# choderalab/openmmtools

Hardware: NVIDIA B200
Metric: replica-exchange iterations/sec, 256-replica alchemical LJ fluid (higher is better)
Workload: dtype f32 dynamics, f64 energies and mixing

## Files before the change

openmmtools_b200/csrc/rx_walk2.cuh:

```cuda
#pragma once

struct SlotRec2 {
    uint32_t ij;
    uint32_t backmask;
    uint32_t lu_next;
    uint32_t alts;
};

#define W2_LOOKBACK 48

__device__ __forceinline__ double slot_logU(const uint32_t *__restrict__ words, unsigned s) {
    const double U = mt_double(words[2 * (size_t)s], words[2 * (size_t)s + 1]);
    return (U == 0.0) ? LOGU_ZERO : log(U);
}

__global__ void __launch_bounds__(256) k_slots_build2(const uint32_t *__restrict__ words, long long nslots, uint32_t mask,
                                                      SlotRec2 *__restrict__ rec) {
    __shared__ uint32_t s_ij[256 + W2_LOOKBACK];
    const long long s0 = (long long)blockIdx.x * 256;
    const int t = threadIdx.x;
    for (int q = t; q < 256 + W2_LOOKBACK; q += 256) {
        const long long s = s0 - W2_LOOKBACK + q;
        uint32_t ij = 0xffffffffu;
        if (s >= 0 && s < nslots) ij = (words[2 * s] & mask) | ((words[2 * s + 1] & mask) << 16);
        s_ij[q] = ij;
    }
    __syncthreads();
    const long long s = s0 + t;
    if (s >= nslots) return;
    const uint32_t ij = s_ij[t + W2_LOOKBACK];
    const uint32_t i = ij & 0xffffu, j = ij >> 16;
    uint32_t bm = 0, a1i = i, a1j = j;
    bool fi = false, fj = false;
#pragma unroll 4
    for (int b = 0; b < W2_LOOKBACK - 1; b++) {
        const uint32_t o = s_ij[t + W2_LOOKBACK - 1 - b];
        const uint32_t oi = o & 0xffffu, oj = o >> 16;
        const bool valid = (o != 0xffffffffu);
        if (b < 31) {
            const bool hit = valid && (oi == i || oi == j || oj == i || oj == j);
            bm |= (hit ? 1u : 0u) << (31 - b);
        }
        if (valid && oi != oj) {
            if (!fi && (oi == i || oj == i)) { a1i = (oi == i) ? oj : oi; fi = true; }
            if (!fj && (oi == j || oj == j)) { a1j = (oi == j) ? oj : oi; fj = true; }
        }
    }
    SlotRec2 r;
    r.ij = ij;
    r.backmask = bm;
    float lu = 0.f;
    if (s + 1 < nslots) lu = (float)slot_logU(words, (unsigned)(s + 1));
    r.lu_next = __float_as_uint(lu);
    r.alts = (a1i & 0xffu) | ((a1j & 0xffu) << 8);
    rec[s] = r;
}

__device__ __forceinline__ void w2_filter(float d_i, float f_ij, float d_j, float f_ji, float e0, float lu,
                                          bool &ge0, bool &acc, bool &undecided) {
    const float lp = (d_i - f_ij) + (d_j - f_ji);
    const float eps = fmaf(fabsf(f_ij) + fabsf(f_ji), 3.2e-5f, e0);
    ge0 = lp > eps;
    const float d = lp - lu;
    const float mar = fmaf(fabsf(lp) + fabsf(lu), 1.3e-7f, eps);
    const bool dec_lp = fabsf(lp) > eps;
    acc = ge0 || (dec_lp && d > mar);
    undecided = !(ge0 || (dec_lp && fabsf(d) > mar));
}

struct __align__(8) W2Replica {
    int state;
    float diag;
};

__device__ __forceinline__ float w2_image(const unsigned short *__restrict__ s_qhi, const unsigned char *__restrict__ s_qlo, unsigned a) {
    return __uint_as_float(__byte_perm((unsigned)s_qhi[a], (unsigned)s_qlo[a], 0x1045));
}

__device__ __forceinline__ uint2 w2_lds64(unsigned a) {
    uint2 v;
    asm volatile("ld.shared.v2.u32 {%0, %1}, [%2];" : "=r"(v.x), "=r"(v.y) : "r"(a) : "memory");
    return v;
}
__device__ __forceinline__ float w2_lds_f32(unsigned a) {
    float v;
    asm("ld.shared.f32 %0, [%1];" : "=f"(v) : "r"(a));
    return v;
}
__device__ __forceinline__ uint4 w2_lds128(unsigned a) {
    uint4 v;
    asm volatile("ld.shared.v4.u32 {%0, %1, %2, %3}, [%4];" : "=r"(v.x), "=r"(v.y), "=r"(v.z), "=r"(v.w) : "r"(a) : "memory");
    return v;
}
__device__ __forceinline__ uint4 w2_lds128_ctx(unsigned a) {
    uint4 v;
    asm("ld.shared.v4.u32 {%0, %1, %2, %3}, [%4];" : "=r"(v.x), "=r"(v.y), "=r"(v.z), "=r"(v.w) : "r"(a));
    return v;
}
__device__ __forceinline__ void w2_sts64(unsigned a, unsigned x, unsigned y) {
    asm volatile("st.shared.v2.u32 [%0], {%1, %2};" ::"r"(a), "r"(x), "r"(y) : "memory");
}
__device__ __forceinline__ unsigned w2_lds32(unsigned a) {
    unsigned v;
    asm volatile("ld.shared.u32 %0, [%1];" : "=r"(v) : "r"(a) : "memory");
    return v;
}
__device__ __forceinline__ float w2_image_at(unsigned a_hi, unsigned a_lo) {
    unsigned hi, lo;
    asm("ld.shared.u16 %0, [%1];" : "=r"(hi) : "r"(a_hi));
    asm("ld.shared.u8 %0, [%1];" : "=r"(lo) : "r"(a_lo));
    return __uint_as_float(__byte_perm(hi, lo, 0x1045));
}

#define W2_RING 512
__device__ __forceinline__ void w2_cp_async16(unsigned dst, const void *src) {
    asm volatile("cp.async.cg.shared.global [%0], [%1], 16;" ::"r"(dst), "l"(src) : "memory");
}
__device__ __forceinline__ void w2_cp_async_commit() { asm volatile("cp.async.commit_group;" ::: "memory"); }
template <int N>
__device__ __forceinline__ void w2_cp_async_wait() { asm volatile("cp.async.wait_group %0;" ::"n"(N) : "memory"); }

__device__ __noinline__ unsigned w2_exact_decision(const SlotRec2 *__restrict__ rec, const uint32_t *__restrict__ words,
                                                   const double *__restrict__ u, unsigned s, unsigned si, unsigned sj, int logK) {
    const unsigned ij = rec[s].ij;
    const unsigned rowi = (ij & 0xffffu) << logK, rowj = (ij >> 16) << logK;
    const double logp = swap_logp(u[rowi | sj], u[rowj | si], u[rowi | si], u[rowj | sj]);
    if (logp >= 0.0) return 3u;
    const unsigned s1 = s + 1;
    const double dd = logp - slot_logU(words, s1);
    bool acc;
    if (dd > 1e-9) acc = true;
    else if (dd < -1e-9) acc = false;
    else acc = mt_double(words[2 * (size_t)s1], words[2 * (size_t)s1 + 1]) < rx_exp_cr(logp);
    return acc ? 2u : 0u;
}

#define W2_THREADS 128
__global__ void __launch_bounds__(W2_THREADS) k_mix_walk2(const SlotRec2 *__restrict__ rec, const uint32_t *__restrict__ words,
                                                  unsigned nslots, const double *__restrict__ u, int K, int logK,
                                                  int *__restrict__ perm_g, uint32_t *__restrict__ slot_log,
                                                  const unsigned char *__restrict__ filt,
                                                  const double *__restrict__ filt_rowabs, MixCtl *ctl) {
    extern __shared__ uint4 s_w2[];
    __shared__ unsigned long long s_ptrs[2];
    uint4 *s_ring = s_w2;
    W2Replica *s_rep = (W2Replica *)(s_ring + W2_RING);
    unsigned char *s_q = (unsigned char *)(s_rep + K);
    const int tid = threadIdx.x, lane = tid & 31, warp = __shfl_sync(0xffffffffu, tid >> 5, 0);
    {
        const unsigned short *ghi = (const unsigned short *)filt;
        const unsigned char *glo = filt + 2 * (size_t)K * K;
        if (K >= 16) {
            const uint4 *ghi4 = (const uint4 *)ghi, *glo4 = (const uint4 *)glo;
            for (int q = tid; q < (K * K) / 8; q += W2_THREADS) {
                const int e = q * 8, row = e >> logK, col = e & (K - 1);
                *(uint4 *)(s_q + (size_t)3 * K * row + 2 * col) = ghi4[q];
            }
            for (int q = tid; q < (K * K) / 16; q += W2_THREADS) {
                const int e = q * 16, row = e >> logK, col = e & (K - 1);
                *(uint4 *)(s_q + (size_t)3 * K * row + 2 * K + col) = glo4[q];
            }
        } else {
            for (int q = tid; q < K * K; q += W2_THREADS) {
                const int row = q >> logK, col = q & (K - 1);
                unsigned char *rowp = s_q + (size_t)3 * K * row;
                ((unsigned short *)rowp)[col] = ghi[q];
                rowp[2 * K + col] = glo[q];
            }
        }
    }
    if (tid == 0) { s_ptrs[0] = (unsigned long long)__cvta_generic_to_global(slot_log); s_ptrs[1] = (unsigned long long)rec; }
    __syncthreads();
    float rowabs_max = 0.f;
    for (int q = tid; q < K; q += W2_THREADS) {
        W2Replica e;
        e.state = perm_g[q];
        const unsigned char *rowp = s_q + (size_t)3 * K * q;
        e.diag = __uint_as_float(__byte_perm((unsigned)((const unsigned short *)rowp)[e.state], (unsigned)rowp[2 * K + e.state], 0x1045));
        s_rep[q] = e;
    }
    for (int q = lane; q < K; q += 32)
        rowabs_max = fmaxf(rowabs_max, __fmul_ru(1.6e-14f, __fadd_ru(__double2float_ru(fabs(filt_rowabs[q])), 0.5f)));
    for (int o = 16; o; o >>= 1) rowabs_max = fmaxf(rowabs_max, __shfl_xor_sync(0xffffffffu, rowabs_max, o));
    const float eps_rows = __fadd_ru(__fadd_ru(rowabs_max, rowabs_max), 1e-9f);
    __syncthreads();
    if (warp != 0) return;
    const uint4 *__restrict__ recs = (const uint4 *)rec;

    const unsigned head0 = (unsigned)ctl->head;
    unsigned h = head0;
    const long long remaining0 = ctl->remaining;
    unsigned rem = remaining0 > 0x7fffffffLL ? 0x7fffffffu : (unsigned)remaining0;
    const unsigned rem0 = rem;
    unsigned rounds = 0, slow = 0;
    const unsigned h_end = nslots >= 1200u ? nslots - 560u : 0u;
    if (rem >= 130 && nslots >= 1200u && h + 99u <= h_end) {
        const unsigned ring_base = __shfl_sync(0xffffffffu, (unsigned)__cvta_generic_to_shared((const void *)s_ring), 0);
        const unsigned rep_base = __shfl_sync(0xffffffffu, (unsigned)__cvta_generic_to_shared((const void *)s_rep), 0);
        const unsigned img_base = __shfl_sync(0xffffffffu, (unsigned)__cvta_generic_to_shared((const void *)s_q), 0);
        const unsigned row_bytes = 3u * (unsigned)K, lo_off = 2u * (unsigned)K;
        unsigned r = h & 31u;
        unsigned w = ((unsigned)lane - h) & 31u;
        unsigned sA = h + w;
        const uint2 pl = w2_lds64((unsigned)__cvta_generic_to_shared((const void *)&s_ptrs[0]));
        const uint2 pr = w2_lds64((unsigned)__cvta_generic_to_shared((const void *)&s_ptrs[1]));
        const unsigned long long slot_log_r = ((unsigned long long)pl.y << 32) | pl.x;
        const uint4 *recs_r = (const uint4 *)(((unsigned long long)pr.y << 32) | pr.x);
        unsigned bmA, neqA, rowiA, rowjA, repiA, repjA;
        float luA, epsA;
        unsigned iB, jB, repiB, repjB;
        auto ahead = [&](const uint4 q) {
            iB = q.x & 0xffffu; jB = q.x >> 16;
            repiB = rep_base + (iB << 3); repjB = rep_base + (jB << 3);
        };
        auto derive = [&](const uint4 q, unsigned &bm, float &lu, float &eps, unsigned &neq, unsigned &rowi, unsigned &rowj,
                          unsigned &repi, unsigned &repj) {
            const unsigned i = q.x & 0xffffu, j = q.x >> 16;
            bm = q.y; lu = __uint_as_float(q.z);
            neq = i != j ? 0xffffffffu : 0u;
            eps = i != j ? eps_rows : -1e30f;
            rowi = img_base + i * row_bytes; rowj = img_base + j * row_bytes;
            repi = rep_base + (i << 3); repj = rep_base + (j << 3);
        };
        for (unsigned k = 0; k < 16u; k++) w2_cp_async16(ring_base + (((sA + 32u * k) & (W2_RING - 1)) << 4), recs + (sA + 32u * k));
        w2_cp_async_commit();
        w2_cp_async_wait<0>();
        __syncwarp();
        derive(w2_lds128(ring_base + ((sA & (W2_RING - 1)) << 4)), bmA, luA, epsA, neqA, rowiA, rowjA, repiA, repjA);
        unsigned ridxB = (sA + 32u) & (W2_RING - 1);
        uint4 qB = w2_lds128(ring_base + (ridxB << 4));
        ahead(qB);
        uint2 ei = w2_lds64(repiA), ej = w2_lds64(repjA);
        unsigned p_cm = 0, p_below = 0, p_chg = 0, p_entry = 0;
        float f_ij = 0.f, f_ji = 0.f;
        auto commit = [&]() {
            const unsigned p_advance = (unsigned)__popc(p_below);
            const unsigned bit = 1u << w;
            const bool p_mine = (p_cm & bit) != 0u;
            const bool p_swaps = (p_cm & bit & p_chg) != 0u;
            const bool p_promoted = (p_below & bit) != 0u;
            if (p_swaps) {
                w2_sts64(repiA, ej.x, __float_as_uint(f_ij));
                w2_sts64(repjA, ei.x, __float_as_uint(f_ji));
            }
            __syncwarp();
            const uint2 ein = w2_lds64(p_promoted ? repiB : repiA), ejn = w2_lds64(p_promoted ? repjB : repjA);
            if (p_mine)
                asm volatile("st.global.u32 [%0], %1;" ::"l"(slot_log_r + 4ull * sA), "r"(p_entry) : "memory");
            if (p_promoted) {
                bmA = qB.y; luA = __uint_as_float(qB.z);
                neqA = iB != jB ? 0xffffffffu : 0u;
                epsA = iB != jB ? eps_rows : -1e30f;
                rowiA = img_base + iB * row_bytes; rowjA = img_base + jB * row_bytes;
                repiA = repiB; repjA = repjB;
                sA += 32u;
                w2_cp_async16(ring_base + (((ridxB - 32u) & (W2_RING - 1)) << 4), recs_r + (sA + 480u));
                ridxB = (ridxB + 32u) & (W2_RING - 1);
            }
            w2_cp_async_commit();
            qB = w2_lds128(ring_base + (ridxB << 4));
            h += p_advance;
            r = (r + p_advance) & 31u;
            rem -= __popc(p_cm);
            ei = ein;
            ej = ejn;
            w = (w - p_advance) & 31u;
        };
        unsigned Cw = 0;
        float bias = 0.f, lu_saved = 0.f;
        bool injected = false;
        for (;;) {
            if (rem < 130u || h + 99u > h_end) break;
            unsigned quota = min(min((rem - 97u) >> 5, (h_end - h - 66u) >> 5), injected ? 1u : 64u);
            do {
                commit();
                rounds++;
                const unsigned si = ei.x, sj = ej.x;
                f_ij = w2_image_at(rowiA + 2u * sj, rowiA + lo_off + sj);
                f_ji = w2_image_at(rowjA + 2u * si, rowjA + lo_off + si);
                const float e0 = fmaf(fabsf(__uint_as_float(ei.y)) + fabsf(__uint_as_float(ej.y)), 3.2e-5f, epsA);
                w2_cp_async_wait<8>();
                ahead(qB);
                bool ge0, acc, undecided;
                w2_filter(__uint_as_float(ei.y), f_ij, __uint_as_float(ej.y) + bias, f_ji, e0, luA, ge0, acc, undecided);
                const unsigned und = undecided ? 1u : 0u;
                const bool changes = acc && neqA != 0u;
                const unsigned G = __ballot_sync(0xffffffffu, ge0);
                const unsigned A = __ballot_sync(0xffffffffu, changes);
                const unsigned Gw = __funnelshift_r(G, G, r), Aw = __funnelshift_r(A, A, r);
                const unsigned X = ~Gw;
                const unsigned starts = X & ~(X << 1);
                const unsigned SE = starts & 0x55555555u, SO = starts & 0xAAAAAAAAu;
                const unsigned sumE = X + SE, sumO = X + SO;
                const unsigned skip = (((sumE ^ X) & ~SE) & 0xAAAAAAAAu) | (((sumO ^ X) & ~SO) & 0x55555555u);
                const unsigned V = ~skip;
                const unsigned VA = V & Aw;
                unsigned earlier;
                asm("shl.b32 %0, %1, %2;" : "=r"(earlier) : "r"(VA), "r"(32u - w));
                const unsigned C = __ballot_sync(0xffffffffu, ((earlier & bmA) | und) != 0u);
                Cw = (__funnelshift_r(C, C, r) | (X & 0x80000000u)) & V;
                const unsigned low = Cw & (0u - Cw);
                const unsigned below = low - 1u;
                p_cm = V & below; p_below = below; p_chg = changes ? 0xffffffffu : 0u;
                p_entry = (sj * (1u << LOG_STATE_BITS) + si) | (acc ? (1u << 31) | (1u << LOG_ACC_BIT) : (1u << 31));
            } while (--quota != 0u && (Cw & 1u) == 0u);
            const bool was_injected = injected;
            luA = was_injected ? lu_saved : luA;
            bias = 0.f;
            injected = false;
            if ((Cw & 1u) == 0u) continue;
            commit();
            w2_cp_async_wait<8>();
            ahead(qB);
            if (!was_injected) {
                const unsigned si = ei.x, sj = ej.x;
                const float f1 = w2_image_at(rowiA + 2u * sj, rowiA + lo_off + sj);
                const float f2 = w2_image_at(rowjA + 2u * si, rowjA + lo_off + si);
                const float e0 = fmaf(fabsf(__uint_as_float(ei.y)) + fabsf(__uint_as_float(ej.y)), 3.2e-5f, epsA);
                bool ge0, acc, undecided;
                w2_filter(__uint_as_float(ei.y), f1, __uint_as_float(ej.y), f2, e0, luA, ge0, acc, undecided);
                lu_saved = luA;
                if (undecided) {
                    const unsigned d = w2_exact_decision(rec, words, u, sA, si, sj, logK);
                    bias = (d & 1u) ? 1e30f : -1e20f;
                    if (!(d & 1u)) luA = (d & 2u) ? -1e30f : 0.f;
                    slow++;
                }
                __syncwarp();
                injected = true;
                continue;
            }
            {
                rounds++;
                bool ge0 = false, acc = false;
                const unsigned si = ei.x, sj = ej.x;
                f_ij = w2_image_at(rowiA + 2u * sj, rowiA + lo_off + sj);
                f_ji = w2_image_at(rowjA + 2u * si, rowjA + lo_off + si);
                if (w == 0u) {
                    const unsigned ij = rec[sA].ij;
                    const unsigned rowi = (ij & 0xffffu) << logK, rowj = (ij >> 16) << logK;
                    const double logp = swap_logp(u[rowi | sj], u[rowj | si], u[rowi | si], u[rowj | sj]);
                    ge0 = logp >= 0.0;
                    acc = ge0;
                    if (!ge0) {
                        const unsigned s1 = sA + 1;
                        const double dd = logp - slot_logU(words, s1);
                        if (dd > 1e-9) acc = true;
                        else if (dd < -1e-9) acc = false;
                        else acc = mt_double(words[2 * (size_t)s1], words[2 * (size_t)s1 + 1]) < rx_exp_cr(logp);
                    }
                    slow++;
                }
                __syncwarp();
                const bool first_ge0 = __ballot_sync(0xffffffffu, ge0) != 0u;
                p_cm = 1u;
                p_below = first_ge0 ? 1u : 3u;
                p_chg = (acc && neqA != 0u) ? 0xffffffffu : 0u;
                p_entry = (sj * (1u << LOG_STATE_BITS) + si) | (acc ? (1u << 31) | (1u << LOG_ACC_BIT) : (1u << 31));
                commit();
                w2_cp_async_wait<8>();
                ahead(qB);
                p_cm = p_below = 0;
            }
        }
        commit();
        w2_cp_async_wait<0>();
        __syncwarp();
        for (int q = lane; q < K; q += 32) perm_g[q] = s_rep[q].state;
    }
    slow = __reduce_add_sync(0xffffffffu, slow);
    if (lane == 0) {
        const long long remaining = remaining0 - (long long)(rem0 - rem);
        ctl->head = h;
        ctl->remaining = remaining;
        ctl->status = remaining > 0 ? 1 : 0;
        ctl->rounds += (int)rounds;
        ctl->slow_exp += slow;
    }
}

__global__ void k_mix_count_slots(const uint32_t *__restrict__ slot_log, long long s0, long long s1, int M,
                                  unsigned long long *__restrict__ nacc, unsigned long long *__restrict__ nprop) {
    long long t = s0 + blockIdx.x * (long long)blockDim.x + threadIdx.x;
    const long long stride = (long long)gridDim.x * blockDim.x;
    for (; t < s1; t += stride) {
        const uint32_t e = slot_log[t];
        if (!(e >> 31)) continue;
        const uint32_t si = e & ((1u << LOG_STATE_BITS) - 1u), sj = (e >> LOG_STATE_BITS) & ((1u << LOG_STATE_BITS) - 1u);
        atomicAdd(&nprop[(size_t)si * M + sj], 1ull);
        atomicAdd(&nprop[(size_t)sj * M + si], 1ull);
        if ((e >> LOG_ACC_BIT) & 1u) {
            atomicAdd(&nacc[(size_t)si * M + sj], 1ull);
            atomicAdd(&nacc[(size_t)sj * M + si], 1ull);
        }
    }
}
```

Baseline: 4.605.

## Speculatively forward single-predecessor swaps in warp-parallel replica mixing walk

The slot precompute now records the offset and side of the nearest earlier slot sharing a replica. The warp walk uses this to evaluate each slot under both outcomes of that one dependency, so a slot whose only conflict is a single accepted predecessor no longer forces the warp to stop and serialize. This adds extra image lookups, a second filter evaluation, another ballot and a two-phase shared-memory commit to every round. The kernel also gets launch_bounds min-blocks of 1, which changes the register budget.

```diff
diff --git a/openmmtools_b200/csrc/rx_walk2.cuh b/openmmtools_b200/csrc/rx_walk2.cuh
--- a/openmmtools_b200/csrc/rx_walk2.cuh
+++ b/openmmtools_b200/csrc/rx_walk2.cuh
@@ -30,7 +30,7 @@
     if (s >= nslots) return;
     const uint32_t ij = s_ij[t + W2_LOOKBACK];
     const uint32_t i = ij & 0xffffu, j = ij >> 16;
-    uint32_t bm = 0, a1i = i, a1j = j;
+    uint32_t bm = 0, a1i = i, a1j = j, offi = 0, offj = 0;
     bool fi = false, fj = false;
 #pragma unroll 4
     for (int b = 0; b < W2_LOOKBACK - 1; b++) {
@@ -42,8 +42,8 @@
             bm |= (hit ? 1u : 0u) << (31 - b);
         }
         if (valid && oi != oj) {
-            if (!fi && (oi == i || oj == i)) { a1i = (oi == i) ? oj : oi; fi = true; }
-            if (!fj && (oi == j || oj == j)) { a1j = (oi == j) ? oj : oi; fj = true; }
+            if (!fi && (oi == i || oj == i)) { a1i = (oi == i) ? oj : oi; offi = b < 31 ? b + 1 : 0; fi = true; }
+            if (!fj && (oi == j || oj == j)) { a1j = (oi == j) ? oj : oi; offj = b < 31 ? b + 1 : 0; fj = true; }
         }
     }
     SlotRec2 r;
@@ -52,7 +52,10 @@
     float lu = 0.f;
     if (s + 1 < nslots) lu = (float)slot_logU(words, (unsigned)(s + 1));
     r.lu_next = __float_as_uint(lu);
-    r.alts = (a1i & 0xffu) | ((a1j & 0xffu) << 8);
+    const bool kj = offi == 0u || (offj != 0u && offj < offi);
+    const uint32_t off = i == j ? 0u : kj ? offj : offi;
+    const bool sw = kj ? a1j == i : a1i == j;
+    r.alts = (a1i & 0xffu) | ((a1j & 0xffu) << 8) | (off << 16) | ((kj ? 1u : 0u) << 24) | ((sw ? 1u : 0u) << 25);
     rec[s] = r;
 }
 
@@ -66,6 +69,21 @@
     const bool dec_lp = fabsf(lp) > eps;
     acc = ge0 || (dec_lp && d > mar);
     undecided = !(ge0 || (dec_lp && fabsf(d) > mar));
+}
+
+__device__ __forceinline__ void w2_filter_pm(float d_i, float f_ij, float d_j, float f_ji, float e0, float lu,
+                                             bool &ge0, bool &acc, bool &undecided, bool &ge0n, bool &accn, bool &undecidedn) {
+    const float lp = (d_i - f_ij) + (d_j - f_ji);
+    const float eps = fmaf(fabsf(f_ij) + fabsf(f_ji), 3.2e-5f, e0);
+    ge0 = lp > eps;
+    ge0n = -lp > eps;
+    const float d = lp - lu, dn = -lp - lu;
+    const float mar = fmaf(fabsf(lp) + fabsf(lu), 1.3e-7f, eps);
+    const bool dec_lp = fabsf(lp) > eps;
+    acc = ge0 || (dec_lp && d > mar);
+    accn = ge0n || (dec_lp && dn > mar);
+    undecided = !(ge0 || (dec_lp && fabsf(d) > mar));
+    undecidedn = !(ge0n || (dec_lp && fabsf(dn) > mar));
 }
 
 struct __align__(8) W2Replica {
@@ -135,8 +153,28 @@
     return acc ? 2u : 0u;
 }
 
+__device__ __forceinline__ unsigned w2_shl(unsigned x, unsigned n) {
+    unsigned y;
+    asm("shl.b32 %0, %1, %2;" : "=r"(y) : "r"(x), "r"(n));
+    return y;
+}
+
+__device__ __forceinline__ unsigned w2_visited(unsigned Gw) {
+    const unsigned X = ~Gw;
+    const unsigned starts = X & ~(X << 1);
+    const unsigned SE = starts & 0x55555555u, SO = starts & 0xAAAAAAAAu;
+    const unsigned sumE = X + SE, sumO = X + SO;
+    return ~((((sumE ^ X) & ~SE) & 0xAAAAAAAAu) | (((sumO ^ X) & ~SO) & 0x55555555u));
+}
+
+__device__ __forceinline__ unsigned w2_sel(bool p, unsigned a, unsigned b) {
+    unsigned y;
+    asm("{ .reg .pred q; setp.ne.u32 q, %1, 0; selp.b32 %0, %2, %3, q; }" : "=r"(y) : "r"((unsigned)p), "r"(a), "r"(b));
+    return y;
+}
+
 #define W2_THREADS 128
-__global__ void __launch_bounds__(W2_THREADS) k_mix_walk2(const SlotRec2 *__restrict__ rec, const uint32_t *__restrict__ words,
+__global__ void __launch_bounds__(W2_THREADS, 1) k_mix_walk2(const SlotRec2 *__restrict__ rec, const uint32_t *__restrict__ words,
                                                   unsigned nslots, const double *__restrict__ u, int K, int logK,
                                                   int *__restrict__ perm_g, uint32_t *__restrict__ slot_log,
                                                   const unsigned char *__restrict__ filt,
@@ -206,12 +244,14 @@
         const uint2 pr = w2_lds64((unsigned)__cvta_generic_to_shared((const void *)&s_ptrs[1]));
         const unsigned long long slot_log_r = ((unsigned long long)pl.y << 32) | pl.x;
         const uint4 *recs_r = (const uint4 *)(((unsigned long long)pr.y << 32) | pr.x);
-        unsigned bmA, neqA, rowiA, rowjA, repiA, repjA;
+        unsigned bmA, neqA, rowiA, rowjA, repiA, repjA, repakA, altsA;
         float luA, epsA;
-        unsigned iB, jB, repiB, repjB;
+        unsigned iB, jB, repiB, repjB, repakB;
+        auto rep_ak = [&](unsigned alts) { return rep_base + (((alts >> ((alts >> 21) & 8u)) & 0xffu) << 3); };
         auto ahead = [&](const uint4 q) {
             iB = q.x & 0xffffu; jB = q.x >> 16;
             repiB = rep_base + (iB << 3); repjB = rep_base + (jB << 3);
+            repakB = rep_ak(q.w);
         };
         auto derive = [&](const uint4 q, unsigned &bm, float &lu, float &eps, unsigned &neq, unsigned &rowi, unsigned &rowj,
                           unsigned &repi, unsigned &repj) {
@@ -226,25 +266,36 @@
         w2_cp_async_commit();
         w2_cp_async_wait<0>();
         __syncwarp();
-        derive(w2_lds128(ring_base + ((sA & (W2_RING - 1)) << 4)), bmA, luA, epsA, neqA, rowiA, rowjA, repiA, repjA);
+        {
+            const uint4 q = w2_lds128(ring_base + ((sA & (W2_RING - 1)) << 4));
+            derive(q, bmA, luA, epsA, neqA, rowiA, rowjA, repiA, repjA);
+            repakA = rep_ak(q.w); altsA = q.w;
+        }
         unsigned ridxB = (sA + 32u) & (W2_RING - 1);
         uint4 qB = w2_lds128(ring_base + (ridxB << 4));
         ahead(qB);
         uint2 ei = w2_lds64(repiA), ej = w2_lds64(repjA);
-        unsigned p_cm = 0, p_below = 0, p_chg = 0, p_entry = 0;
-        float f_ij = 0.f, f_ji = 0.f;
+        unsigned sak = w2_lds32(repakA);
+        unsigned p_cm = 0, p_below = 0, p_chg = 0, p_fwd = 0, p_entry = 0, p_sti = 0, p_stj = 0;
+        float p_dgi = 0.f, p_dgj = 0.f;
         auto commit = [&]() {
             const unsigned p_advance = (unsigned)__popc(p_below);
             const unsigned bit = 1u << w;
             const bool p_mine = (p_cm & bit) != 0u;
             const bool p_swaps = (p_cm & bit & p_chg) != 0u;
             const bool p_promoted = (p_below & bit) != 0u;
-            if (p_swaps) {
-                w2_sts64(repiA, ej.x, __float_as_uint(f_ij));
-                w2_sts64(repjA, ei.x, __float_as_uint(f_ji));
+            if (p_swaps && p_fwd == 0u) {
+                w2_sts64(repiA, p_sti, __float_as_uint(p_dgi));
+                w2_sts64(repjA, p_stj, __float_as_uint(p_dgj));
+            }
+            __syncwarp();
+            if (p_swaps && p_fwd != 0u) {
+                w2_sts64(repiA, p_sti, __float_as_uint(p_dgi));
+                w2_sts64(repjA, p_stj, __float_as_uint(p_dgj));
             }
             __syncwarp();
             const uint2 ein = w2_lds64(p_promoted ? repiB : repiA), ejn = w2_lds64(p_promoted ? repjB : repjA);
+            const unsigned sakn = w2_lds32(p_promoted ? repakB : repakA);
             if (p_mine)
                 asm volatile("st.global.u32 [%0], %1;" ::"l"(slot_log_r + 4ull * sA), "r"(p_entry) : "memory");
             if (p_promoted) {
@@ -253,6 +304,7 @@
                 epsA = iB != jB ? eps_rows : -1e30f;
                 rowiA = img_base + iB * row_bytes; rowjA = img_base + jB * row_bytes;
                 repiA = repiB; repjA = repjB;
+                repakA = repakB; altsA = qB.w;
                 sA += 32u;
                 w2_cp_async16(ring_base + (((ridxB - 32u) & (W2_RING - 1)) << 4), recs_r + (sA + 480u));
                 ridxB = (ridxB + 32u) & (W2_RING - 1);
@@ -264,6 +316,7 @@
             rem -= __popc(p_cm);
             ei = ein;
             ej = ejn;
+            sak = sakn;
             w = (w - p_advance) & 31u;
         };
         unsigned Cw = 0;
@@ -276,33 +329,52 @@
                 commit();
                 rounds++;
                 const unsigned si = ei.x, sj = ej.x;
-                f_ij = w2_image_at(rowiA + 2u * sj, rowiA + lo_off + sj);
-                f_ji = w2_image_at(rowjA + 2u * si, rowjA + lo_off + si);
-                const float e0 = fmaf(fabsf(__uint_as_float(ei.y)) + fabsf(__uint_as_float(ej.y)), 3.2e-5f, epsA);
+                const float d_i = __uint_as_float(ei.y), d_j = __uint_as_float(ej.y);
+                const float f_ij = w2_image_at(rowiA + 2u * sj, rowiA + lo_off + sj);
+                const float f_ji = w2_image_at(rowjA + 2u * si, rowjA + lo_off + si);
+                const float x_i = w2_image_at(rowiA + 2u * sak, rowiA + lo_off + sak);
+                const float x_j = w2_image_at(rowjA + 2u * sak, rowjA + lo_off + sak);
+                const float e0 = fmaf(fabsf(d_i) + fabsf(d_j), 3.2e-5f, epsA);
                 w2_cp_async_wait<8>();
                 ahead(qB);
-                bool ge0, acc, undecided;
-                w2_filter(__uint_as_float(ei.y), f_ij, __uint_as_float(ej.y) + bias, f_ji, e0, luA, ge0, acc, undecided);
-                const unsigned und = undecided ? 1u : 0u;
+                const bool kj = (altsA >> 24) & 1u;
+                const float fd_i = __uint_as_float(w2_sel(kj, __float_as_uint(d_i), __float_as_uint(x_i)));
+                const float ff_ij = __uint_as_float(w2_sel(kj, __float_as_uint(x_i), __float_as_uint(f_ij)));
+                const float fd_j = __uint_as_float(w2_sel(kj, __float_as_uint(x_j), __float_as_uint(d_j)));
+                const float ff_ji = __uint_as_float(w2_sel(kj, __float_as_uint(f_ji), __float_as_uint(x_j)));
+                const bool sw = (altsA >> 25) & 1u;
+                bool g0, a0, u0, gf, af, uf;
+                {
+                    bool g1, a1, u1, g2, a2, u2;
+                    w2_filter_pm(d_i, f_ij, d_j + bias, f_ji, e0, luA, g0, a0, u0, g2, a2, u2);
+                    w2_filter(fd_i, ff_ij, fd_j, ff_ji, fmaf(fabsf(fd_i) + fabsf(fd_j), 3.2e-5f, epsA), luA, g1, a1, u1);
+                    gf = sw ? g2 : g1; af = sw ? a2 : a1; uf = sw ? u2 : u1;
+                }
+                const unsigned T = injected ? 0u : w2_shl(1u, 32u - ((altsA >> 16) & 0xffu));
+                const unsigned G0 = __ballot_sync(0xffffffffu, g0);
+                const unsigned A0 = __ballot_sync(0xffffffffu, a0 && neqA != 0u);
+                const unsigned VA0 = w2_visited(__funnelshift_r(G0, G0, r)) & __funnelshift_r(A0, A0, r);
+                const unsigned S0 = w2_shl(VA0, 32u - w) & bmA;
+                const bool fwd0 = S0 != 0u && S0 == T, bad0 = S0 != 0u && !fwd0;
+                const bool ge0 = fwd0 ? gf : g0, acc = fwd0 ? af : a0;
                 const bool changes = acc && neqA != 0u;
                 const unsigned G = __ballot_sync(0xffffffffu, ge0);
                 const unsigned A = __ballot_sync(0xffffffffu, changes);
-                const unsigned Gw = __funnelshift_r(G, G, r), Aw = __funnelshift_r(A, A, r);
-                const unsigned X = ~Gw;
-                const unsigned starts = X & ~(X << 1);
-                const unsigned SE = starts & 0x55555555u, SO = starts & 0xAAAAAAAAu;
-                const unsigned sumE = X + SE, sumO = X + SO;
-                const unsigned skip = (((sumE ^ X) & ~SE) & 0xAAAAAAAAu) | (((sumO ^ X) & ~SO) & 0x55555555u);
-                const unsigned V = ~skip;
-                const unsigned VA = V & Aw;
-                unsigned earlier;
-                asm("shl.b32 %0, %1, %2;" : "=r"(earlier) : "r"(VA), "r"(32u - w));
-                const unsigned C = __ballot_sync(0xffffffffu, ((earlier & bmA) | und) != 0u);
-                Cw = (__funnelshift_r(C, C, r) | (X & 0x80000000u)) & V;
+                const unsigned F = __ballot_sync(0xffffffffu, fwd0);
+                const unsigned Gw = __funnelshift_r(G, G, r), Aw = __funnelshift_r(A, A, r), Fw = __funnelshift_r(F, F, r);
+                const unsigned V = w2_visited(Gw);
+                const unsigned S1 = w2_shl(V & Aw, 32u - w) & bmA;
+                const bool fwd1 = S1 != 0u && S1 == T && (S1 & w2_shl(Fw, 32u - w)) == 0u, bad1 = S1 != 0u && !fwd1;
+                const unsigned C = __ballot_sync(0xffffffffu, bad0 || bad1 || fwd0 != fwd1 || (fwd1 ? uf : u0));
+                Cw = (__funnelshift_r(C, C, r) | (~Gw & 0x80000000u)) & V;
                 const unsigned low = Cw & (0u - Cw);
                 const unsigned below = low - 1u;
-                p_cm = V & below; p_below = below; p_chg = changes ? 0xffffffffu : 0u;
-                p_entry = (sj * (1u << LOG_STATE_BITS) + si) | (acc ? (1u << 31) | (1u << LOG_ACC_BIT) : (1u << 31));
+                p_cm = V & below; p_below = below; p_chg = changes ? 0xffffffffu : 0u; p_fwd = fwd0 ? 1u : 0u;
+                p_sti = w2_sel(fwd0, w2_sel(sw, si, w2_sel(kj, sak, sj)), sj);
+                p_stj = w2_sel(fwd0, w2_sel(sw, sj, w2_sel(kj, si, sak)), si);
+                p_dgi = __uint_as_float(w2_sel(fwd0, w2_sel(sw, __float_as_uint(d_i), __float_as_uint(ff_ij)), __float_as_uint(f_ij)));
+                p_dgj = __uint_as_float(w2_sel(fwd0, w2_sel(sw, __float_as_uint(d_j), __float_as_uint(ff_ji)), __float_as_uint(f_ji)));
+                p_entry = (p_sti * (1u << LOG_STATE_BITS) + p_stj) | (acc ? (1u << 31) | (1u << LOG_ACC_BIT) : (1u << 31));
             } while (--quota != 0u && (Cw & 1u) == 0u);
             const bool was_injected = injected;
             luA = was_injected ? lu_saved : luA;
@@ -334,8 +406,9 @@
                 rounds++;
                 bool ge0 = false, acc = false;
                 const unsigned si = ei.x, sj = ej.x;
-                f_ij = w2_image_at(rowiA + 2u * sj, rowiA + lo_off + sj);
-                f_ji = w2_image_at(rowjA + 2u * si, rowjA + lo_off + si);
+                p_dgi = w2_image_at(rowiA + 2u * sj, rowiA + lo_off + sj);
+                p_dgj = w2_image_at(rowjA + 2u * si, rowjA + lo_off + si);
+                p_sti = sj; p_stj = si; p_fwd = 0u;
                 if (w == 0u) {
                     const unsigned ij = rec[sA].ij;
                     const unsigned rowi = (ij & 0xffffu) << logK, rowj = (ij >> 16) << logK;
```

After: 3.361 (median of 6 runs). 27.0% lower.
